# Graylab/DFMDock

Measured on AMD Instinct MI355X. Metric: docking trajectories/sec (N_res~300+300, 40 steps), higher is better.
Workload: dtype f16

## Files before the change

### dfmdock_amd/csrc/kernels_dense.hip

```cpp
#include <cstdlib>
#include "dfm_device.h"
#include "dfm_internal.h"

namespace dfm {

typedef float f32x16 __attribute__((ext_vector_type(16)));

constexpr int BM = 128, BN = 128, BK = 16, LDT = BM + 1;

__global__ __launch_bounds__(256) void k_gemm_f32(GemmArgs a)
{
    __shared__ float As[BK * LDT];
    __shared__ float Ws[BK * LDT];
    const int tid = threadIdx.x, lane = tid & 63, wave = tid >> 6;
    const int wm = wave >> 1, wn = wave & 1;
    const int row0 = blockIdx.x * BM, col0 = blockIdx.y * BN;

    f32x16 acc[2][2];
#pragma unroll
    for (int i = 0; i < 2; ++i)
#pragma unroll
        for (int j = 0; j < 2; ++j)
#pragma unroll
            for (int r = 0; r < 16; ++r) acc[i][j][r] = 0.f;

    const int lr = tid >> 2;
    const int lk = (tid & 3) * 4;
    const int halfK = a.K >> 1;

    for (int k0 = 0; k0 < a.K; k0 += BK) {
#pragma unroll
        for (int rr = 0; rr < 2; ++rr) {
            const int r = lr + rr * 64;
            const int grow = row0 + r;
            const int grow_a = a.a0_period ? grow % a.a0_period : grow;
            float v[4] = {0.f, 0.f, 0.f, 0.f};
            if (grow < a.M) {
#pragma unroll
                for (int e = 0; e < 4; ++e) {
                    const int k = k0 + lk + e;
                    if (k < a.K) {
                        float x;
                        if (a.pro == 1) {
                            x = (k < halfK) ? a.A0[(size_t)grow_a * a.lda + k] : a.A1[(size_t)grow * a.lda + (k - halfK)];
                        } else {
                            x = a.A0[(size_t)grow_a * a.lda + k];
                            if (a.pro == 2) {
                                const int g = grow / a.rows_per_graph;
                                const float o = x - a.gn_shift[(size_t)g * H + k];
                                x = silu_exact(a.gn_w[k] * o / a.gn_den[(size_t)g * H + k] + a.gn_b[k]);
                            } else if (a.pro == 3) {
                                x = silu_exact(x);
                            }
                        }
                        v[e] = x;
                    }
                }
            }
#pragma unroll
            for (int e = 0; e < 4; ++e) As[(lk + e) * LDT + r] = v[e];
            const int gcol = col0 + r;
            float w[4] = {0.f, 0.f, 0.f, 0.f};
            if (gcol < a.Nout) {
#pragma unroll
                for (int e = 0; e < 4; ++e) {
                    const int k = k0 + lk + e;
                    if (k < a.K) w[e] = a.W[(size_t)gcol * a.ldw + k];
                }
            }
#pragma unroll
            for (int e = 0; e < 4; ++e) Ws[(lk + e) * LDT + r] = w[e];
        }
        __syncthreads();
#pragma unroll
        for (int kk = 0; kk < BK; kk += 2) {
            const int k = kk + (lane >> 5);
            float af[2], bf[2];
#pragma unroll
            for (int i = 0; i < 2; ++i) af[i] = As[k * LDT + wm * 64 + i * 32 + (lane & 31)];
#pragma unroll
            for (int j = 0; j < 2; ++j) bf[j] = Ws[k * LDT + wn * 64 + j * 32 + (lane & 31)];
#pragma unroll
            for (int i = 0; i < 2; ++i)
#pragma unroll
                for (int j = 0; j < 2; ++j)
                    acc[i][j] = __builtin_amdgcn_mfma_f32_32x32x2f32(af[i], bf[j], acc[i][j], 0, 0, 0);
        }
        __syncthreads();
    }

#pragma unroll
    for (int i = 0; i < 2; ++i)
#pragma unroll
        for (int j = 0; j < 2; ++j) {
            const int col = col0 + wn * 64 + j * 32 + (lane & 31);
            if (col >= a.Nout) continue;
            const float bias = a.bias ? a.bias[col] : 0.f;
#pragma unroll
            for (int r = 0; r < 16; ++r) {
                const int row = row0 + wm * 64 + i * 32 + (r & 3) + 8 * (r >> 2) + 4 * (lane >> 5);
                if (row >= a.M) continue;
                float v = acc[i][j][r] + bias;
                if (a.epi == 1) {
                    a.C[(size_t)row * a.ldc + col] = a.R[(size_t)(a.r_period ? row % a.r_period : row) * a.ldc + col] + v;
                } else if (a.epi == 2) {
                    if (col < H) a.C[(size_t)row * H + col] = v;
                    else {
                        a.C2[(size_t)row * H + (col - H)] = v;
                        if (a.C2b) a.C2b[(size_t)row * H + (col - H)] = f2h(v);
                    }
                } else {
                    a.C[(size_t)row * a.ldc + col] = v;
                }
            }
        }
}

__global__ __launch_bounds__(256) void k_gemm_f32v(GemmArgs a)
{
    __shared__ float As[2][BK * LDT];
    __shared__ float Ws[2][BK * LDT];
    const int tid = threadIdx.x, lane = tid & 63, wave = tid >> 6;
    const int wm = wave >> 1, wn = wave & 1;
    const int row0 = blockIdx.x * BM, col0 = blockIdx.y * BN;
    f32x16 acc[2][2];
#pragma unroll
    for (int i = 0; i < 2; ++i)
#pragma unroll
        for (int j = 0; j < 2; ++j)
#pragma unroll
            for (int r = 0; r < 16; ++r) acc[i][j][r] = 0.f;
    const int lr = tid >> 2, lk = (tid & 3) * 4;
    const int halfK = a.K >> 1;
    int grow[2], gcol[2];
    size_t arow0[2], arow1[2];
    bool rv[2], cv[2];
#pragma unroll
    for (int rr = 0; rr < 2; ++rr) {
        grow[rr] = row0 + lr + rr * 64; gcol[rr] = col0 + lr + rr * 64;
        rv[rr] = grow[rr] < a.M; cv[rr] = gcol[rr] < a.Nout;
        const int g = rv[rr] ? grow[rr] : 0;
        arow0[rr] = (size_t)(a.a0_period ? g % a.a0_period : g) * a.lda;
        arow1[rr] = (size_t)g * a.lda;
    }
    float4 ra[2], rw[2];
    auto fetch = [&](int k0) {
#pragma unroll
        for (int rr = 0; rr < 2; ++rr) {
            const int k = k0 + lk;
            const float *src = (a.pro == 1 && k >= halfK) ? a.A1 + arow1[rr] + (k - halfK) : a.A0 + arow0[rr] + k;
            ra[rr] = *reinterpret_cast<const float4 *>(src);
            rw[rr] = *reinterpret_cast<const float4 *>(a.W + (size_t)(cv[rr] ? gcol[rr] : 0) * a.ldw + k);
        }
    };
    auto stage = [&](int k0, int buf) {
#pragma unroll
        for (int rr = 0; rr < 2; ++rr) {
            const int r = lr + rr * 64;
            float v[4] = {ra[rr].x, ra[rr].y, ra[rr].z, ra[rr].w};
            if (a.pro == 2) {
                const int g = (rv[rr] ? grow[rr] : 0) / a.rows_per_graph;
#pragma unroll
                for (int e = 0; e < 4; ++e) {
                    const int k = k0 + lk + e;
                    const float o = v[e] - a.gn_shift[(size_t)g * H + k];
                    v[e] = silu_exact(a.gn_w[k] * o / a.gn_den[(size_t)g * H + k] + a.gn_b[k]);
                }
            } else if (a.pro == 3) {
#pragma unroll
                for (int e = 0; e < 4; ++e) v[e] = silu_exact(v[e]);
            }
#pragma unroll
            for (int e = 0; e < 4; ++e) As[buf][(lk + e) * LDT + r] = rv[rr] ? v[e] : 0.f;
            const float w[4] = {rw[rr].x, rw[rr].y, rw[rr].z, rw[rr].w};
#pragma unroll
            for (int e = 0; e < 4; ++e) Ws[buf][(lk + e) * LDT + r] = cv[rr] ? w[e] : 0.f;
        }
    };
    fetch(0);
    int buf = 0;
    for (int k0 = 0; k0 < a.K; k0 += BK, buf ^= 1) {
        stage(k0, buf);
        __syncthreads();
        if (k0 + BK < a.K) fetch(k0 + BK);
#pragma unroll
        for (int kk = 0; kk < BK; kk += 2) {
            const int k = kk + (lane >> 5);
            float af[2], bf[2];
#pragma unroll
            for (int i = 0; i < 2; ++i) af[i] = As[buf][k * LDT + wm * 64 + i * 32 + (lane & 31)];
#pragma unroll
            for (int j = 0; j < 2; ++j) bf[j] = Ws[buf][k * LDT + wn * 64 + j * 32 + (lane & 31)];
#pragma unroll
            for (int i = 0; i < 2; ++i)
#pragma unroll
                for (int j = 0; j < 2; ++j)
                    acc[i][j] = __builtin_amdgcn_mfma_f32_32x32x2f32(af[i], bf[j], acc[i][j], 0, 0, 0);
        }
    }
#pragma unroll
    for (int i = 0; i < 2; ++i)
#pragma unroll
        for (int j = 0; j < 2; ++j) {
            const int col = col0 + wn * 64 + j * 32 + (lane & 31);
            if (col >= a.Nout) continue;
            const float bias = a.bias ? a.bias[col] : 0.f;
#pragma unroll
            for (int r = 0; r < 16; ++r) {
                const int row = row0 + wm * 64 + i * 32 + (r & 3) + 8 * (r >> 2) + 4 * (lane >> 5);
                if (row >= a.M) continue;
                float v = acc[i][j][r] + bias;
                if (a.epi == 1) {
                    a.C[(size_t)row * a.ldc + col] = a.R[(size_t)(a.r_period ? row % a.r_period : row) * a.ldc + col] + v;
                } else if (a.epi == 2) {
                    if (col < H) a.C[(size_t)row * H + col] = v;
                    else {
                        a.C2[(size_t)row * H + (col - H)] = v;
                        if (a.C2b) a.C2b[(size_t)row * H + (col - H)] = f2h(v);
                    }
                } else {
                    a.C[(size_t)row * a.ldc + col] = v;
                }
            }
        }
}

hipError_t launch_gemm_f32(const GemmArgs &a, hipStream_t s)
{
    const dim3 grid((a.M + BM - 1) / BM, (a.Nout + BN - 1) / BN);
    const bool aligned = a.K % BK == 0 && a.lda % 4 == 0 && a.ldw % 4 == 0 && (a.pro != 1 || (a.K / 2) % 4 == 0) &&
                         ((uintptr_t)a.A0 % 16 == 0) && ((uintptr_t)a.W % 16 == 0) && (a.pro != 1 || (uintptr_t)a.A1 % 16 == 0);
    if (aligned) hipLaunchKernelGGL(k_gemm_f32v, grid, dim3(256), 0, s, a);
    else hipLaunchKernelGGL(k_gemm_f32, grid, dim3(256), 0, s, a);
    return hipGetLastError();
}

constexpr int GN_CH = 20;
__device__ inline void gn_finish_col(const float *__restrict__ part, int b, int N, int c, const float *__restrict__ mean_scale,
                                     const float *__restrict__ fold_w, const float *__restrict__ fold_b, float &o_den, float &o_shift)
{
    const int tpt = (N + 31) / 32;
    const float *base = part + (size_t)b * tpt * (H * 2) + c * 2;
    double S1 = 0, S2 = 0, SM = 0;
    for (int t0 = 0; t0 < tpt; t0 += GN_CH) {
        float2 v[GN_CH];
#pragma unroll
        for (int u = 0; u < GN_CH; ++u) {
            const int t = t0 + u < tpt ? t0 + u : tpt - 1;
            v[u] = *reinterpret_cast<const float2 *>(base + (size_t)t * (H * 2));
        }
#pragma unroll
        for (int u = 0; u < GN_CH; ++u) {
            const int t = t0 + u;
            if (t < tpt) {
                const double nt = (double)(N - t * 32 < 32 ? N - t * 32 : 32), m = (double)v[u].x, w = nt * m;
                S1 += w; S2 += w * m; SM += (double)v[u].y;
            }
        }
    }
    const double mean = S1 / N;
    const double M2 = SM + (S2 - mean * S1);
    const float sft = (float)mean * mean_scale[c];
    const double dm = mean - (double)sft;
    double var = M2 / N + dm * dm;
    var = var > 0 ? var : 0;
    const float dn = sqrtf((float)var + 1e-5f);
    if (fold_w) {
        const float sc = fold_w[c] / dn;
        o_den = sc;
        o_shift = fold_b[c] - sc * sft;
    } else {
        o_shift = sft;
        o_den = dn;
    }
}

typedef __bf16 bf16x8 __attribute__((ext_vector_type(8)));
union FragB { uint4 u; bf16x8 b; };
constexpr int SK = 32, SLD = 40;

struct GemmSplitArgs {
    GemmArgs g;
    const uint16_t *Whi, *Wlo;
};

__device__ inline uint32_t pack2(__bf16 a, __bf16 b)
{
    union { __bf16 h[2]; uint32_t u; } v;
    v.h[0] = a; v.h[1] = b;
    return v.u;
}

template <int HALF, int NJ, int QT = 0, int RING = QT> __global__ __launch_bounds__(256, RING ? 1 : 3) void k_gemm_split(GemmSplitArgs sa)
{
    static_assert(!QT || NJ == 1, "quarter tiles: one 32-column tile per wave");
    static_assert(!RING || NJ == 1, "the register ring is sized for the 64 x 128 and 64 x 64 shapes");
    static_assert(!QT || RING, "quarter tiles always run the ring");
    constexpr int MI = QT ? 1 : 2;
    constexpr int SM = 64, SN = QT ? 64 : NJ * 128;
    const GemmArgs &a = sa.g;
#ifdef DFM_GEMM_STAMP
    const unsigned long long g_entry = __builtin_amdgcn_s_memtime(), g_rt0 = __builtin_amdgcn_s_memrealtime();
#endif
    constexpr int LDS_BUF = (2 * SM + 2 * SN) * SLD;
    constexpr int LDS_OPER = (RING ? 2 : 1) * LDS_BUF, LDS_EPI = 4 * 32 * 72 * 2;
    constexpr int LDS_U16 = LDS_OPER > LDS_EPI ? LDS_OPER : LDS_EPI;
    __shared__ __attribute__((aligned(16))) uint16_t lds[LDS_U16];
    uint16_t *Ah = lds, *Al = lds + SM * SLD, *Wh = lds + 2 * SM * SLD, *Wl = lds + (2 * SM + SN) * SLD;
    const int tid = threadIdx.x, lane = tid & 63, wave = tid >> 6;
    const int wm = QT ? wave >> 1 : 0, wn = QT ? wave & 1 : wave, l31 = lane & 31;
    __shared__ __attribute__((aligned(16))) float gn_s[2 * H];
    const int vb = blockIdx.x;
    int bx = vb, by = blockIdx.y;
    if (NJ == 2 && gridDim.y == 1 && a.Nout == 2 * SN) {
        const int g16 = bx >> 4, j = bx & 15;
        bx = g16 * 8 + (j & 7); by = j >> 3;
        if (bx * SM >= a.M) return;
    }
    int row0 = bx * SM, row_end = a.M, gn_tb = 0;
    const int col0 = by * SN;
    if (a.stat_part || a.pro == 2) {
        const int tpt = (a.rows_per_graph + SM - 1) / SM, tb = bx / tpt;
        row0 = tb * a.rows_per_graph + (bx - tb * tpt) * SM;
        row_end = (tb + 1) * a.rows_per_graph;
        gn_tb = tb;
    }
    if (a.zbuf) {
        const int zr = tid >> 2;
        if (row0 + zr < row_end) {
            float4 *z = reinterpret_cast<float4 *>(a.zbuf + (size_t)(row0 + zr) * H + col0 + (tid & 3) * (SN / 4));
#pragma unroll
            for (int q = 0; q < SN / 16; ++q) z[q] = make_float4(0.f, 0.f, 0.f, 0.f);
        }
    }
    constexpr int LPR = SN * 4 / 128, NTOUCH = QT ? (SM * LPR + 255) / 256 : 0;
    float touch[NTOUCH + 1];
#pragma unroll
    for (int q = 0; q < NTOUCH; ++q) {
        touch[q] = 0.f;
        const int t = tid + q * 256, row = row0 + t / LPR;
        if (a.epi == 1 && t < SM * LPR && row < row_end) {
            const int rrow = a.r_period ? row % a.r_period : row;
            touch[q] = a.R[(size_t)rrow * a.ldc + col0 + (t % LPR) * 32];
        }
    }
    f32x16 acc[MI][NJ];
#pragma unroll
    for (int i = 0; i < MI; ++i)
#pragma unroll
        for (int j = 0; j < NJ; ++j)
#pragma unroll
            for (int r = 0; r < 16; ++r) acc[i][j][r] = 0.f;

    const int ar = tid >> 2, kg = (tid & 3) * 8;
    const int halfK = a.K >> 1;
    const bool rv0 = row0 + ar < row_end;
    const size_t gr0 = (size_t)(rv0 ? row0 + ar : 0);
    const size_t gr0a = a.a0_period ? gr0 % (size_t)a.a0_period : gr0;

    float4 xa0, xa1;
    uint4 wh0, wh1, wh2, wh3, wl0, wl1, wl2, wl3;
    const int wcol = QT ? (tid & 63) : (NJ == 2 ? tid : (tid & 127));
    const int wkq = QT ? (tid >> 7) * 2 : 0;
    const uint16_t *wsrc = QT ? (((tid >> 6) & 1) ? sa.Wlo : sa.Whi) : ((NJ == 2 || tid < 128) ? sa.Whi : sa.Wlo);
#define GEMM_SPLIT_FETCH(K0)                                                                                          \
    {                                                                                                                 \
        const int k_ = (K0) + kg;                                                                                     \
        const bool second_ = a.pro == 1 && k_ >= halfK;                                                               \
        const float *s0_ = second_ ? a.A1 + (k_ - halfK) + gr0 * a.lda : a.A0 + k_ + gr0a * a.lda;                    \
        xa0 = *reinterpret_cast<const float4 *>(s0_); xa1 = *reinterpret_cast<const float4 *>(s0_ + 4);              \
        const size_t wbase_ = ((size_t)((K0) / SK) * 4 * a.Nout + col0 + wcol) * 8;                                   \
        const size_t wq_ = (size_t)a.Nout * 8;                                                                        \
        const uint16_t *ph_ = wsrc + wbase_ + wkq * wq_, *pl_ = sa.Wlo + wbase_;                                      \
        wh0 = *reinterpret_cast<const uint4 *>(ph_); wh1 = *reinterpret_cast<const uint4 *>(ph_ + wq_);               \
        if constexpr (!QT) {                                                                                          \
            wh2 = *reinterpret_cast<const uint4 *>(ph_ + 2 * wq_); wh3 = *reinterpret_cast<const uint4 *>(ph_ + 3 * wq_); \
        }                                                                                                             \
        if constexpr (NJ == 2) {                                                                                      \
            wl0 = *reinterpret_cast<const uint4 *>(pl_); wl1 = *reinterpret_cast<const uint4 *>(pl_ + wq_);               \
            wl2 = *reinterpret_cast<const uint4 *>(pl_ + 2 * wq_); wl3 = *reinterpret_cast<const uint4 *>(pl_ + 3 * wq_); \
        }                                                                                                             \
    }
    auto stage_row = [&](const float4 &v0, const float4 &v1, bool , int k, int row, int boff = 0) {
        float x[8] = {v0.x, v0.y, v0.z, v0.w, v1.x, v1.y, v1.z, v1.w};
        if (a.pro == 2) {
            const float4 c0 = *reinterpret_cast<const float4 *>(&gn_s[k]), c1 = *reinterpret_cast<const float4 *>(&gn_s[k + 4]);
            const float4 h0 = *reinterpret_cast<const float4 *>(&gn_s[H + k]), h1 = *reinterpret_cast<const float4 *>(&gn_s[H + k + 4]);
            const float cc[8] = {c0.x, c0.y, c0.z, c0.w, c1.x, c1.y, c1.z, c1.w};
            const float hh[8] = {h0.x, h0.y, h0.z, h0.w, h1.x, h1.y, h1.z, h1.w};
#pragma unroll
            for (int e = 0; e < 8; ++e) {
                const float y = fmaf(x[e], cc[e], hh[e]);
                x[e] = y * __builtin_amdgcn_rcpf(1.0f + __expf(-y));
            }
        }
        uint32_t hi[4], lo[4];
#pragma unroll
        for (int e = 0; e < 4; ++e) {
            const float x0 = x[2 * e], x1 = x[2 * e + 1];
            const __bf16 b0 = (__bf16)x0, b1 = (__bf16)x1;
            hi[e] = pack2(b0, b1);
            lo[e] = pack2((__bf16)(x0 - (float)b0), (__bf16)(x1 - (float)b1));
        }
        *reinterpret_cast<uint4 *>(&Ah[boff + row * SLD + kg]) = make_uint4(hi[0], hi[1], hi[2], hi[3]);
        *reinterpret_cast<uint4 *>(&Al[boff + row * SLD + kg]) = make_uint4(lo[0], lo[1], lo[2], lo[3]);
    };

    const int wu = wcol * SLD + wkq * 8;
    uint16_t *wdst = QT ? (((tid >> 6) & 1) ? Wl : Wh) : ((NJ == 2 || tid < 128) ? Wh : Wl);
#ifdef DFM_GEMM_STAMP
    unsigned long long gs[4] = {0, 0, 0, 0}, gprev = __builtin_amdgcn_s_memtime();
    const unsigned long long g_first = gprev;
#define GSTAMP(k) { __builtin_amdgcn_sched_barrier(0); const unsigned long long _n = __builtin_amdgcn_s_memtime(); gs[k] += _n - gprev; gprev = _n; __builtin_amdgcn_sched_barrier(0); }
#else
#define GSTAMP(k)
#endif
    float bias_r[NJ];
#pragma unroll
    for (int j = 0; j < NJ; ++j) bias_r[j] = a.bias ? a.bias[col0 + (wn * NJ + j) * 32 + l31] : 0.f;
    constexpr int QD = RING ? 4 : 1, RW = QT ? 2 : 4;
    float4 rxa0[QD], rxa1[QD];
    uint4 rw[QD][RW];
    GEMM_SPLIT_FETCH(0)
#define RING_TAKE(d) { rxa0[d] = xa0; rxa1[d] = xa1; rw[d][0] = wh0; rw[d][1] = wh1; if constexpr (!QT) { rw[d][2] = wh2; rw[d][3] = wh3; } }
#define RING_WSTORE(d, nb) { _Pragma("unroll") for (int q_ = 0; q_ < RW; ++q_) *reinterpret_cast<uint4 *>(&wdst[(nb) + wu + 8 * q_]) = rw[d][q_]; }
    if constexpr (RING) {
        RING_TAKE(0)
#pragma unroll
        for (int d = 1; d < QD; ++d) {
            GEMM_SPLIT_FETCH((d * SK < a.K ? d : 0) * SK)
            RING_TAKE(d)
        }
    }
    if (a.pro == 2) {
        if (a.gn_part) {
            float sc, sh;
            gn_finish_col(a.gn_part, gn_tb, a.rows_per_graph, tid, a.gn_ms, a.gn_w, a.gn_b, sc, sh);
            gn_s[tid] = sc; gn_s[H + tid] = sh;
        } else if (tid < 128) {
            const float *src = (tid < 64 ? a.gn_den : a.gn_shift) + (size_t)gn_tb * H + (tid & 63) * 4;
            *reinterpret_cast<float4 *>(&gn_s[(tid < 64 ? 0 : H) + (tid & 63) * 4]) = *reinterpret_cast<const float4 *>(src);
        }
        __syncthreads();
    }
    auto mfma_stage = [&](int boff = 0) {
#pragma unroll
        for (int ks = 0; ks < SK; ks += 16) {
            const int ko = ks + (lane >> 5) * 8;
            FragB ah[MI], al[MI];
#pragma unroll
            for (int i = 0; i < MI; ++i) {
                const int r = (wm * MI + i) * 32 + l31;
                ah[i].u = *reinterpret_cast<const uint4 *>(&Ah[boff + r * SLD + ko]);
                al[i].u = *reinterpret_cast<const uint4 *>(&Al[boff + r * SLD + ko]);
            }
#pragma unroll
            for (int j = 0; j < NJ; ++j) {
                const int c = (wn * NJ + j) * 32 + l31;
                FragB wh, wl;
                wh.u = *reinterpret_cast<const uint4 *>(&Wh[boff + c * SLD + ko]);
                wl.u = *reinterpret_cast<const uint4 *>(&Wl[boff + c * SLD + ko]);
#pragma unroll
                for (int i = 0; i < MI; ++i) {
                    acc[i][j] = __builtin_amdgcn_mfma_f32_32x32x16_bf16(al[i].b, wh.b, acc[i][j], 0, 0, 0);
                    acc[i][j] = __builtin_amdgcn_mfma_f32_32x32x16_bf16(ah[i].b, wl.b, acc[i][j], 0, 0, 0);
                    acc[i][j] = __builtin_amdgcn_mfma_f32_32x32x16_bf16(ah[i].b, wh.b, acc[i][j], 0, 0, 0);
                }
            }
        }
    };
    if constexpr (RING) {
        const int S = a.K / SK;
        stage_row(rxa0[0], rxa1[0], rv0, kg, ar, 0);
        RING_WSTORE(0, 0)
        {
            GEMM_SPLIT_FETCH((QD < S ? QD : S - 1) * SK)
            RING_TAKE(0)
        }
        __syncthreads();
        GSTAMP(1)
        for (int k0 = 0; k0 < S; k0 += QD) {
#pragma unroll
            for (int d = 0; d < QD; ++d) {
                const int k = k0 + d;
                const int dn = (d + 1) % QD, nb = ((d + 1) & 1) * LDS_BUF;
                const int kn = k + 1 < S ? k + 1 : S - 1, kf = k + 1 + QD < S ? k + 1 + QD : S - 1;
                mfma_stage((d & 1) * LDS_BUF);
                GSTAMP(0)
                stage_row(rxa0[dn], rxa1[dn], rv0, kn * SK + kg, ar, nb);
                RING_WSTORE(dn, nb)
                {
                    GEMM_SPLIT_FETCH(kf * SK)
                    RING_TAKE(dn)
                }
                GSTAMP(1)
                __syncthreads();
                GSTAMP(2)
            }
        }
    } else {
        for (int k0 = 0; k0 < a.K; k0 += SK) {
            if (k0) __syncthreads();
            GSTAMP(0)
            stage_row(xa0, xa1, rv0, k0 + kg, ar);
            *reinterpret_cast<uint4 *>(&wdst[wu]) = wh0; *reinterpret_cast<uint4 *>(&wdst[wu + 8]) = wh1;
            if constexpr (!QT) { *reinterpret_cast<uint4 *>(&wdst[wu + 16]) = wh2; *reinterpret_cast<uint4 *>(&wdst[wu + 24]) = wh3; }
            if constexpr (NJ == 2) {
                *reinterpret_cast<uint4 *>(&Wl[wu]) = wl0; *reinterpret_cast<uint4 *>(&Wl[wu + 8]) = wl1;
                *reinterpret_cast<uint4 *>(&Wl[wu + 16]) = wl2; *reinterpret_cast<uint4 *>(&Wl[wu + 24]) = wl3;
            }
            GSTAMP(1)
            __syncthreads();
            GSTAMP(2)
            if (k0 + SK < a.K) GEMM_SPLIT_FETCH(k0 + SK)
            mfma_stage();
        }
    }
#pragma unroll
    for (int q = 0; q < NTOUCH; ++q) asm volatile("" :: "v"(touch[q]));
    GSTAMP(0)
    __syncthreads();
    constexpr int ELD = 72;
    float *est = reinterpret_cast<float *>(lds) + wave * (32 * ELD);
    const int er = lane >> 4, ec = (lane & 15) * 4;
    float st_s[MI][4], st_q[MI][4], st_p[MI][4], st_n[MI];
#pragma unroll
    for (int i = 0; i < MI; ++i) {
        st_n[i] = 0.f;
#pragma unroll
        for (int e = 0; e < 4; ++e) { st_s[i][e] = 0.f; st_q[i][e] = 0.f; st_p[i][e] = 0.f; }
    }
#pragma unroll
    for (int i = 0; i < MI; ++i)
#pragma unroll
        for (int jp = 0; jp < (NJ + 1) / 2; ++jp) {
            float4 res[8];
            if (a.epi == 1) {
#pragma unroll
                for (int q = 0; q < 8; ++q) {
                    const size_t row = (size_t)row0 + (wm * MI + i) * 32 + q * 4 + er;
                    const size_t rrow = a.r_period ? row % (size_t)a.r_period : row;
                    const int col = col0 + (wn * NJ + jp * 2) * 32 + ec;
                    res[q] = (row < (size_t)row_end && ec < NJ * 32) ? *reinterpret_cast<const float4 *>(a.R + rrow * a.ldc + col) : make_float4(0.f, 0.f, 0.f, 0.f);
                }
            }
#pragma unroll
            for (int jj = 0; jj < (NJ < 2 ? NJ : 2); ++jj) {
                const int j = jp * 2 + jj;
                const float bias = bias_r[j];
#pragma unroll
                for (int r = 0; r < 16; ++r)
                    est[((r & 3) + 8 * (r >> 2) + 4 * (lane >> 5)) * ELD + jj * 32 + l31] = acc[i][j][r] + bias;
            }
            asm volatile("s_waitcnt lgkmcnt(0)" ::: "memory");
            if constexpr (HALF) {
                uint16_t *half_out = col0 < H ? a.Cb : a.C2b;
                const int er8 = lane >> 3, ec8 = (lane & 7) * 8;
#pragma unroll
                for (int q = 0; q < 4; ++q) {
                    const int lr = q * 8 + er8;
                    const float4 v0 = *reinterpret_cast<const float4 *>(est + lr * ELD + ec8);
                    const float4 v1 = *reinterpret_cast<const float4 *>(est + lr * ELD + ec8 + 4);
                    const size_t row = (size_t)row0 + (wm * MI + i) * 32 + lr;
                    const int col = (col0 < H ? col0 : col0 - H) + (wn * NJ + jp * 2) * 32 + ec8;
                    if (row >= (size_t)row_end || ec8 >= NJ * 32) continue;
                    uint4 o;
                    o.x = pack_h2_sat(v0.x, v0.y); o.y = pack_h2_sat(v0.z, v0.w);
                    o.z = pack_h2_sat(v1.x, v1.y); o.w = pack_h2_sat(v1.z, v1.w);
                    *reinterpret_cast<uint4 *>(half_out + row * H + col) = o;
                }
            } else {
#pragma unroll
            for (int q = 0; q < 8; ++q) {
                const int lr = q * 4 + er;
                const float4 v = *reinterpret_cast<const float4 *>(est + lr * ELD + ec);
                const size_t row = (size_t)row0 + (wm * MI + i) * 32 + lr;
                const int col = col0 + (wn * NJ + jp * 2) * 32 + ec;
                if (row >= (size_t)row_end || ec >= NJ * 32) continue;
                {
                    if (a.stat_part) {
#pragma clang fp contract(off)
                        if (st_n[i] == 0.f) { st_p[i][0] = v.x; st_p[i][1] = v.y; st_p[i][2] = v.z; st_p[i][3] = v.w; }
                        const float d0 = v.x - st_p[i][0], d1 = v.y - st_p[i][1], d2 = v.z - st_p[i][2], d3 = v.w - st_p[i][3];
                        st_s[i][0] += d0; st_s[i][1] += d1; st_s[i][2] += d2; st_s[i][3] += d3;
                        st_q[i][0] += d0 * d0; st_q[i][1] += d1 * d1; st_q[i][2] += d2 * d2; st_q[i][3] += d3 * d3;
                        st_n[i] += 1.f;
                    }
                }
                if (a.epi == 1) {
                    const float4 rr = res[q];
                    *reinterpret_cast<float4 *>(a.C + row * a.ldc + col) = make_float4(rr.x + v.x, rr.y + v.y, rr.z + v.z, rr.w + v.w);
                } else if (a.epi == 2) {
                    if (col0 < H) {
                        if (a.Cb) {
                            uint2 o;
                            o.x = pack_h2_sat(v.x, v.y);
                            o.y = pack_h2_sat(v.z, v.w);
                            *reinterpret_cast<uint2 *>(a.Cb + row * H + col) = o;
                        } else *reinterpret_cast<float4 *>(a.C + row * H + col) = v;
                    } else {
                        if (a.C2) *reinterpret_cast<float4 *>(a.C2 + row * H + (col - H)) = v;
                        if (a.C2b) {
                            uint2 o;
                            o.x = pack_h2_sat(v.x, v.y);
                            o.y = pack_h2_sat(v.z, v.w);
                            *reinterpret_cast<uint2 *>(a.C2b + row * H + (col - H)) = o;
                        }
                    }
                } else {
                    *reinterpret_cast<float4 *>(a.C + row * a.ldc + col) = v;
                }
            }
            }
            asm volatile("s_waitcnt lgkmcnt(0)" ::: "memory");
        }
    if (a.stat_part) {
#pragma clang fp contract(off)
        const int tpt64 = (a.rows_per_graph + 63) / 64, tpt32 = (a.rows_per_graph + 31) / 32;
#pragma unroll
        for (int i = 0; i < MI; ++i) {
            const int sub = (vb % tpt64) * 2 + wm * MI + i;
            float *sp = a.stat_part + ((size_t)(vb / tpt64) * tpt32 + sub) * (H * 2);
            const float inv_n = st_n[i] > 0.f ? 1.0f / st_n[i] : 0.f;
            float nl[2], fl[2];
            {
                float ne = st_n[i];
#pragma unroll
                for (int lv = 0; lv < 2; ++lv) {
                    const float n2 = __shfl_xor(ne, 16 << lv, 64), nt = ne + n2;
                    nl[lv] = ne;
                    fl[lv] = nt > 0.f ? n2 / nt : 0.f;
                    ne = nt;
                }
            }
#pragma unroll
            for (int e = 0; e < 4; ++e) {
                float mean = st_p[i][e] + st_s[i][e] * inv_n, M2 = st_q[i][e] - st_s[i][e] * st_s[i][e] * inv_n;
#pragma unroll
                for (int lv = 0; lv < 2; ++lv) {
                    const float mean2 = __shfl_xor(mean, 16 << lv, 64), M22 = __shfl_xor(M2, 16 << lv, 64);
                    const float d = mean2 - mean, f = fl[lv];
                    mean += d * f;
                    M2 += M22 + d * d * nl[lv] * f;
                }
                if (er == 0 && ec < NJ * 32 && sub < tpt32) {
                    const int c = col0 + wn * (NJ * 32) + ec + e;
                    sp[c * 2] = mean;
                    sp[c * 2 + 1] = M2;
                }
            }
        }
    }
#ifdef DFM_GEMM_STAMP
    GSTAMP(3)
    if (vb == (gridDim.x > 2048 ? 7 * 8 + 1536 : 3) && blockIdx.y == 0 && tid == 0 && a.C) {
        const unsigned long long g_rt1 = __builtin_amdgcn_s_memrealtime();
        printf("gemm stamp K=%d Nout=%d pro=%d epi=%d stats=%d gn=%d: entry->loop %llu  mfma+barrier %llu  fetch-wait+stage %llu  barrier2 %llu  epilogue %llu  total %llu shader cycles in %llu ticks of 100 MHz = %llu MHz\n",
               a.K, a.Nout, a.pro, a.epi, a.stat_part ? 1 : 0, a.gn_part ? 1 : 0, g_first - g_entry, gs[0], gs[1], gs[2], gs[3], gprev - g_entry, g_rt1 - g_rt0,
               (g_rt1 > g_rt0) ? 100ull * (gprev - g_entry) / (g_rt1 - g_rt0) : 0ull);
    }
#endif
}
#undef GEMM_SPLIT_FETCH

int gemm_rows_per_tile() { return 64; }

hipError_t launch_gemm_split(const GemmArgs &a, const uint16_t *Whi, const uint16_t *Wlo, hipStream_t s)
{
    constexpr int SN = 256;
    if (a.K % SK != 0 || a.Nout % SN != 0 || (a.pro == 1 && (a.K / 2) % SK != 0) || a.lda % 4 != 0 || a.ldc % 4 != 0)
        return hipErrorInvalidValue;
    GemmSplitArgs sa;
    sa.g = a; sa.Whi = Whi; sa.Wlo = Wlo;
    if (a.stat_part && (a.Nout != SN || a.rows_per_graph < 1 || a.M % a.rows_per_graph != 0)) return hipErrorInvalidValue;
    if (a.pro == 2 && (a.rows_per_graph < 1 || a.M % a.rows_per_graph != 0)) return hipErrorInvalidValue;
    if (a.zbuf && a.Nout != SN) return hipErrorInvalidValue;
    const int row_tiles = (a.stat_part || a.pro == 2) ? (a.M / a.rows_per_graph) * ((a.rows_per_graph + 63) / 64) : (a.M + 63) / 64;
    static const int narrow_env = [] {
        const char *e = getenv("DFM_GEMM_NARROW_MAXWG");
        return e ? atoi(e) : -1;
    }();
    const int narrow_max = narrow_env >= 0 ? narrow_env : 2 * device_cus();
    const bool narrow = (long long)row_tiles * (a.Nout / SN) < narrow_max;
    const bool half = a.epi == 2 && a.Cb && a.C2b && !a.C2;
    if (narrow) {
        static const int quarter_env = [] {
            const char *e = getenv("DFM_GEMM_QUARTER_MAXWG");
            return e ? atoi(e) : -1;
        }();
        const int quarter_max = quarter_env >= 0 ? quarter_env : device_cus() / 2;
        if ((long long)row_tiles * (a.Nout / 128) < quarter_max && (a.K / 32) % 4 == 0) {
            const dim3 grid(row_tiles, a.Nout / 64);
            if (half) hipLaunchKernelGGL((k_gemm_split<1, 1, 1>), grid, dim3(256), 0, s, sa);
            else hipLaunchKernelGGL((k_gemm_split<0, 1, 1>), grid, dim3(256), 0, s, sa);
            return hipGetLastError();
        }
        const dim3 grid(row_tiles, a.Nout / 128);
        if (half) hipLaunchKernelGGL((k_gemm_split<1, 1>), grid, dim3(256), 0, s, sa);
        else hipLaunchKernelGGL((k_gemm_split<0, 1>), grid, dim3(256), 0, s, sa);
        return hipGetLastError();
    }
    dim3 grid;
    if (a.stat_part || a.pro == 2) grid = dim3(row_tiles, a.Nout / SN);
    else if (a.Nout == 2 * SN) grid = dim3((((a.M + 63) / 64 + 7) / 8) * 16, 1);
    else grid = dim3((a.M + 63) / 64, a.Nout / SN);
    if (half) hipLaunchKernelGGL((k_gemm_split<1, 2>), grid, dim3(256), 0, s, sa);
    else hipLaunchKernelGGL((k_gemm_split<0, 2>), grid, dim3(256), 0, s, sa);
    return hipGetLastError();
}

__global__ __launch_bounds__(256) void k_gn_stats(const float *__restrict__ u, int N, const float *__restrict__ mean_scale,
                                                  float *__restrict__ shift, float *__restrict__ den,
                                                  const float *__restrict__ fold_w, const float *__restrict__ fold_b)
{
    __shared__ double red[16][64];
    __shared__ float sh_shift[64];
    const int b = blockIdx.x, cq = threadIdx.x & 15, rl = threadIdx.x >> 4, c0 = blockIdx.y * 64;
    const float *U = u + (size_t)b * N * H + c0 + cq * 4;
    auto reduce_rows = [&](const double (&s)[4]) {
#pragma unroll
        for (int e = 0; e < 4; ++e) red[rl][cq * 4 + e] = s[e];
        __syncthreads();
        if (threadIdx.x < 64) {
            double t = 0;
#pragma unroll
            for (int r = 0; r < 16; ++r) t += red[r][threadIdx.x];
            red[0][threadIdx.x] = t;
        }
        __syncthreads();
    };
    double s[4] = {0, 0, 0, 0};
    for (int n = rl; n < N; n += 16) {
        const float4 v = *reinterpret_cast<const float4 *>(U + (size_t)n * H);
        s[0] += v.x; s[1] += v.y; s[2] += v.z; s[3] += v.w;
    }
    reduce_rows(s);
    if (threadIdx.x < 64) sh_shift[threadIdx.x] = (float)(red[0][threadIdx.x] / N) * mean_scale[c0 + threadIdx.x];
    __syncthreads();
    const float4 sft = *reinterpret_cast<const float4 *>(&sh_shift[cq * 4]);
    double v2[4] = {0, 0, 0, 0};
    for (int n = rl; n < N; n += 16) {
        const float4 v = *reinterpret_cast<const float4 *>(U + (size_t)n * H);
        const float o0 = v.x - sft.x, o1 = v.y - sft.y, o2 = v.z - sft.z, o3 = v.w - sft.w;
        v2[0] += (double)o0 * o0; v2[1] += (double)o1 * o1; v2[2] += (double)o2 * o2; v2[3] += (double)o3 * o3;
    }
    reduce_rows(v2);
    if (threadIdx.x < 64) {
        const int c = c0 + threadIdx.x;
        const float var = (float)(red[0][threadIdx.x] / N);
        const float dn = sqrtf(var + 1e-5f), sf = sh_shift[threadIdx.x];
        if (fold_w) {
            const float sc = fold_w[c] / dn;
            den[(size_t)b * H + c] = sc;
            shift[(size_t)b * H + c] = fold_b[c] - sc * sf;
        } else {
            shift[(size_t)b * H + c] = sf;
            den[(size_t)b * H + c] = dn;
        }
    }
}

hipError_t launch_gn_stats(const float *u, int B, int N, const float *mean_scale, float *shift, float *den,
                           const float *fold_w, const float *fold_b, hipStream_t s)
{
    hipLaunchKernelGGL(k_gn_stats, dim3(B, 4), dim3(256), 0, s, u, N, mean_scale, shift, den, fold_w, fold_b);
    return hipGetLastError();
}

}
```

Measured before the change: 445.0.

## Prefetch activations two K-stages ahead in wide split GEMM path

Result: no change. 447.6, median of 6 (+0.6%).

```diff
diff --git a/dfmdock_amd/csrc/kernels_dense.hip b/dfmdock_amd/csrc/kernels_dense.hip
--- a/dfmdock_amd/csrc/kernels_dense.hip
+++ b/dfmdock_amd/csrc/kernels_dense.hip
@@ -278,6 +278,7 @@
 typedef __bf16 bf16x8 __attribute__((ext_vector_type(8)));
 union FragB { uint4 u; bf16x8 b; };
 constexpr int SK = 32, SLD = 40;
+constexpr int GEMM_ACT_DEPTH = 2;
 
 struct GemmSplitArgs {
     GemmArgs g;
@@ -363,12 +364,15 @@
     const int wcol = QT ? (tid & 63) : (NJ == 2 ? tid : (tid & 127));
     const int wkq = QT ? (tid >> 7) * 2 : 0;
     const uint16_t *wsrc = QT ? (((tid >> 6) & 1) ? sa.Wlo : sa.Whi) : ((NJ == 2 || tid < 128) ? sa.Whi : sa.Wlo);
-#define GEMM_SPLIT_FETCH(K0)                                                                                          \
+#define GEMM_SPLIT_FETCH_A(K0)                                                                                        \
     {                                                                                                                 \
         const int k_ = (K0) + kg;                                                                                     \
         const bool second_ = a.pro == 1 && k_ >= halfK;                                                               \
         const float *s0_ = second_ ? a.A1 + (k_ - halfK) + gr0 * a.lda : a.A0 + k_ + gr0a * a.lda;                    \
         xa0 = *reinterpret_cast<const float4 *>(s0_); xa1 = *reinterpret_cast<const float4 *>(s0_ + 4);              \
+    }
+#define GEMM_SPLIT_FETCH_W(K0)                                                                                        \
+    {                                                                                                                 \
         const size_t wbase_ = ((size_t)((K0) / SK) * 4 * a.Nout + col0 + wcol) * 8;                                   \
         const size_t wq_ = (size_t)a.Nout * 8;                                                                        \
         const uint16_t *ph_ = wsrc + wbase_ + wkq * wq_, *pl_ = sa.Wlo + wbase_;                                      \
@@ -381,6 +385,7 @@
             wl2 = *reinterpret_cast<const uint4 *>(pl_ + 2 * wq_); wl3 = *reinterpret_cast<const uint4 *>(pl_ + 3 * wq_); \
         }                                                                                                             \
     }
+#define GEMM_SPLIT_FETCH(K0) { GEMM_SPLIT_FETCH_A(K0) GEMM_SPLIT_FETCH_W(K0) }
     auto stage_row = [&](const float4 &v0, const float4 &v1, bool , int k, int row, int boff = 0) {
         float x[8] = {v0.x, v0.y, v0.z, v0.w, v1.x, v1.y, v1.z, v1.w};
         if (a.pro == 2) {
@@ -430,6 +435,16 @@
         for (int d = 1; d < QD; ++d) {
             GEMM_SPLIT_FETCH((d * SK < a.K ? d : 0) * SK)
             RING_TAKE(d)
+        }
+    }
+    constexpr int AD = NJ == 2 ? GEMM_ACT_DEPTH : 1;
+    float4 ra0[AD], ra1[AD];
+    if constexpr (NJ == 2) {
+        ra0[0] = xa0; ra1[0] = xa1;
+#pragma unroll
+        for (int d = 1; d < AD; ++d) {
+            GEMM_SPLIT_FETCH_A((d * SK < a.K ? d : a.K / SK - 1) * SK)
+            ra0[d] = xa0; ra1[d] = xa1;
         }
     }
     if (a.pro == 2) {
@@ -496,6 +511,28 @@
                 GSTAMP(1)
                 __syncthreads();
                 GSTAMP(2)
+            }
+        }
+    } else if constexpr (NJ == 2) {
+        const int S = a.K / SK;
+        for (int s0 = 0; s0 < S; s0 += AD) {
+#pragma unroll
+            for (int d = 0; d < AD; ++d) {
+                const int s = s0 + d;
+                GSTAMP(0)
+                stage_row(ra0[d], ra1[d], rv0, s * SK + kg, ar);
+                *reinterpret_cast<uint4 *>(&Wh[wu]) = wh0; *reinterpret_cast<uint4 *>(&Wh[wu + 8]) = wh1;
+                *reinterpret_cast<uint4 *>(&Wh[wu + 16]) = wh2; *reinterpret_cast<uint4 *>(&Wh[wu + 24]) = wh3;
+                *reinterpret_cast<uint4 *>(&Wl[wu]) = wl0; *reinterpret_cast<uint4 *>(&Wl[wu + 8]) = wl1;
+                *reinterpret_cast<uint4 *>(&Wl[wu + 16]) = wl2; *reinterpret_cast<uint4 *>(&Wl[wu + 24]) = wl3;
+                GSTAMP(1)
+                __syncthreads();
+                GSTAMP(2)
+                GEMM_SPLIT_FETCH_W((s + 1 < S ? s + 1 : S - 1) * SK)
+                GEMM_SPLIT_FETCH_A((s + AD < S ? s + AD : S - 1) * SK)
+                ra0[d] = xa0; ra1[d] = xa1;
+                mfma_stage();
+                __syncthreads();
             }
         }
     } else {
@@ -662,6 +699,8 @@
 #endif
 }
 #undef GEMM_SPLIT_FETCH
+#undef GEMM_SPLIT_FETCH_A
+#undef GEMM_SPLIT_FETCH_W
 
 int gemm_rows_per_tile() { return 64; }
 
@@ -681,7 +720,7 @@
         return e ? atoi(e) : -1;
     }();
     const int narrow_max = narrow_env >= 0 ? narrow_env : 2 * device_cus();
-    const bool narrow = (long long)row_tiles * (a.Nout / SN) < narrow_max;
+    const bool narrow = (long long)row_tiles * (a.Nout / SN) < narrow_max || (a.K / SK) % GEMM_ACT_DEPTH != 0;
     const bool half = a.epi == 2 && a.Cb && a.C2b && !a.C2;
     if (narrow) {
         static const int quarter_env = [] {
```
